# ltronchin/Gan-track

Hardware: AMD Instinct MI355X
Metric: imgs/sec at 256^2 bs32/GPU StyleGAN2-ADA training (+ sec/kimg) (higher is better)
Workload: dtype fp16+fp32 (fp16 at the 4 highest resolutions, fp32 below; f32 accumulate); 1 GPU; StyleGAN2-ADA train iteration, 256x256 1-ch, c_dim 2, cbase 16384, map 8, Gmain+Dmain / Greg every 4 / Dreg every 16, ADA geometric p=0.2; global_batch=32, batch_gpu=32, resolution=256, parallelism=dp1

## Files before the change

### gan-track_amd/csrc/conv3x3.hip

```cpp
#include "sg2_common.h"

#include <algorithm>
#include <atomic>
#include <type_traits>

namespace sg2 {
namespace {

constexpr int CK = 32;
constexpr int BN = 64;
constexpr int PX = CK;

__device__ __forceinline__ int swz64(int p, int q) { return p * 64 + ((q ^ ((p >> 1) & 2)) << 4); }

struct Conv3Args {
    const void* x;
    const void* w;
    void* y;
    void* y_raw;
    const float* in_scale;
    const float* out_scale;
    const void* noise;
    const float* bias;
    const void* dot_src;
    float* dot_out;
    float noise_gain, alpha, gain, clamp;
    int act;
    int N, H, W, Cin, Cout;
    int tiles_x, tiles_y;
    int OH, OW;
    const void* residual;
    int raw_act;
    float* det_dot;
    int edge_rx, edge_cy;
    int det_maxb;
};

__device__ __forceinline__ int p_chan(int P) { return (P >> 5) * 32 + 8 * ((P & 15) >> 2) + 4 * ((P >> 4) & 1) + (P & 3); }

template <typename T>
using v8 = typename std::conditional<std::is_same<T, bf16_t>::value, bf16x8, f16x8>::type;

template <typename T>
__device__ __forceinline__ f32x4 mma(v8<T> a, v8<T> b, f32x4 c) {
    if constexpr (std::is_same<T, bf16_t>::value)
        return __builtin_amdgcn_mfma_f32_16x16x32_bf16(a, b, c, 0, 0, 0);
    else
        return __builtin_amdgcn_mfma_f32_16x16x32_f16(a, b, c, 0, 0, 0);
}

template <typename T, int TW, bool SCALE_IN, bool EPI, int NBUF, int S = 1, bool DIR = false>
__global__ __launch_bounds__(256, 3 - NBUF) void conv3x3_halo_kernel(Conv3Args a) {
    static_assert(!DIR || S == 1, "the direct epilogue is the stride-1 form");
    constexpr int TH = S == 1 ? 256 / TW : 4;
    constexpr int PXW = TW * TH / 4, NFR = PXW / 16;
    constexpr int HW_ = S * (TW - 1) + 3, HH = S * (TH - 1) + 3, HP = HW_ * HH;
    constexpr int HEV = (HW_ + 1) / 2;
    constexpr int HALO = HP * PX;
    constexpr int WTS = 9 * BN * PX;
    constexpr int NH = (HP * 4 + 255) / 256;
    constexpr int NW = (9 * BN * 4) / 256;
    typedef T vec8 __attribute__((ext_vector_type(8)));

    extern __shared__ __attribute__((aligned(16))) char smem_raw[];
    T* smem = (T*)smem_raw;

    const int tid = threadIdx.x, lane = tid & 63, wave = tid >> 6;
    const int tile = blockIdx.x;
    const int n = tile / (a.tiles_x * a.tiles_y);
    const int tr = tile - n * a.tiles_x * a.tiles_y;
    const int ty0 = (tr / a.tiles_x) * TH, tx0 = (tr % a.tiles_x) * TW;
    const int o0 = blockIdx.y * BN;
    const T* __restrict__ x = (const T*)a.x;
    const T* __restrict__ w = (const T*)a.w;
    const int nchunks = (a.Cin + CK - 1) / CK;

    int h_src[NH], h_dst[NH];
    bool h_ok[NH];
#pragma unroll
    for (int i = 0; i < NH; ++i) {
        const int idx = tid + i * 256;
        const int p = idx >> 2, q = idx & 3;
        const int hy = p / HW_, hx = p - hy * HW_;
        const int iy = S == 1 ? ty0 - 1 + hy : 2 * ty0 + hy, ix = S == 1 ? tx0 - 1 + hx : 2 * tx0 + hx;
        h_ok[i] = p < HP && iy >= 0 && iy < a.H && ix >= 0 && ix < a.W;
        h_src[i] = h_ok[i] ? ((n * a.H + iy) * a.W + ix) : 0;
        const int pl = S == 1 ? p : hy * HW_ + ((hx & 1) ? HEV + (hx >> 1) : (hx >> 1));
        h_dst[i] = p < HP ? swz64(pl, q) : -1;
    }
    const int hq = (tid & 3) * 8;
    int w_src[NW], w_dst[NW];
    bool w_ok[NW];
#pragma unroll
    for (int i = 0; i < NW; ++i) {
        const int idx = tid + i * 256;
        const int r = idx >> 2;
        const int tap = r / BN, o = r - tap * BN;
        w_ok[i] = o0 + o < a.Cout;
        w_src[i] = (w_ok[i] ? (o0 + (DIR ? p_chan(o) : o)) : 0) * 9 + tap;
        w_dst[i] = swz64(tap * BN + o, idx & 3);
    }

    const __amdgpu_buffer_rsrc_t rxb = make_rsrc(x, (int64_t)a.N * a.H * a.W * a.Cin * (int64_t)sizeof(T));
    const __amdgpu_buffer_rsrc_t rwb = make_rsrc(w, (int64_t)a.Cout * 9 * a.Cin * (int64_t)sizeof(T));
    vec8 rh[NH], rw[NW];
    float4 sc0, sc1;
    auto gload = [&](int chunk) {
        const int c = chunk * CK + hq;
        const bool cok = c < a.Cin;
        const int cc = cok ? c : 0;
#pragma unroll
        for (int i = 0; i < NH; ++i)
            rh[i] = buf_load16<vec8>(rxb, h_ok[i] && cok ? (h_src[i] * a.Cin + c) * (int)sizeof(T) : -1);
#pragma unroll
        for (int i = 0; i < NW; ++i)
            rw[i] = buf_load16<vec8>(rwb, w_ok[i] && cok ? (w_src[i] * a.Cin + c) * (int)sizeof(T) : -1);
        if (SCALE_IN) {
            const float* sc = a.in_scale + (int64_t)n * a.Cin + cc;
            sc0 = *(const float4*)sc;
            sc1 = *(const float4*)(sc + 4);
        }
    };
    auto sstore = [&](int buf) {
        T* hb = smem + buf * (HALO + WTS);
        T* wb = hb + HALO;
        const float scl[8] = {sc0.x, sc0.y, sc0.z, sc0.w, sc1.x, sc1.y, sc1.z, sc1.w};
#pragma unroll
        for (int i = 0; i < NH; ++i) {
            if (h_dst[i] < 0) continue;
            vec8 v = rh[i];
            if (SCALE_IN) {
#pragma unroll
                for (int j = 0; j < 8; ++j) v[j] = (T)((float)v[j] * (float)(T)scl[j]);
            }
            *(vec8*)((char*)hb + h_dst[i]) = v;
        }
#pragma unroll
        for (int i = 0; i < NW; ++i) *(vec8*)((char*)wb + w_dst[i]) = rw[i];
    };

    const int lq = lane >> 4, l16 = lane & 15;
    int a_pos[NFR];
#pragma unroll
    for (int i = 0; i < NFR; ++i) {
        const int m = wave * PXW + i * 16 + l16;
        const int py = m / TW, px = m - py * TW;
        a_pos[i] = S * py * HW_ + px;
    }
    const int b_lane = swz64(l16, lq);

    f32x4 acc[NFR][4];
#pragma unroll
    for (int i = 0; i < NFR; ++i)
#pragma unroll
        for (int j = 0; j < 4; ++j) acc[i][j] = f32x4{0.f, 0.f, 0.f, 0.f};

    gload(0);
    sstore(0);
    __syncthreads();
    for (int ch = 0; ch < nchunks; ++ch) {
        const int cur = NBUF == 2 ? (ch & 1) : 0;
        const bool more = ch + 1 < nchunks;
        if (more) gload(ch + 1);
        const char* hb = (const char*)(smem + cur * (HALO + WTS));
        const char* wb = hb + HALO * sizeof(T) + b_lane;
#pragma unroll
        for (int ky = 0; ky < 3; ++ky) {
#pragma unroll
            for (int kx = 0; kx < 3; ++kx) {
                const int tap = ky * 3 + kx;
                const int toff = ky * HW_ + (S == 1 ? kx : ((kx & 1) ? HEV : (kx >> 1)));
                v8<T> af[NFR], bfr[4];
#pragma unroll
                for (int i = 0; i < NFR; ++i) af[i] = *(const v8<T>*)(hb + swz64(a_pos[i] + toff, lq));
#pragma unroll
                for (int j = 0; j < 4; ++j) bfr[j] = *(const v8<T>*)(wb + (tap * BN + j * 16) * 64);
#pragma unroll
                for (int i = 0; i < NFR; ++i)
#pragma unroll
                    for (int j = 0; j < 4; ++j) acc[i][j] = DIR ? mma<T>(bfr[j], af[i], acc[i][j]) : mma<T>(af[i], bfr[j], acc[i][j]);
            }
        }
        if (NBUF == 1 && more) __syncthreads();
        if (more) sstore(NBUF == 2 ? (cur ^ 1) : 0);
        __syncthreads();
    }

    if constexpr (DIR) {
        float dsc[2][8], bsc[2][8];
#pragma unroll
        for (int h = 0; h < 2; ++h)
#pragma unroll
            for (int e = 0; e < 8; ++e) {
                const int o = o0 + 32 * h + 8 * lq + e;
                dsc[h][e] = (EPI && a.out_scale) ? a.out_scale[(int64_t)n * a.Cout + o] : 1.f;
                bsc[h][e] = (EPI && a.bias) ? (float)(T)a.bias[o] : 0.f;
            }
        typedef T vec8d __attribute__((ext_vector_type(8)));
        const bool want_dot = a.dot_out != nullptr, atom = want_dot && !a.det_dot;
        float* red = (float*)smem;
        if (atom) {
            if (tid < BN) red[tid] = 0.f;
            __syncthreads();
        }
        float dacc[2][8];
#pragma unroll
        for (int h = 0; h < 2; ++h)
#pragma unroll
            for (int e = 0; e < 8; ++e) dacc[h][e] = 0.f;
        T* y = (T*)a.y;
        T* yr = (T*)a.y_raw;
        const T* dsrc = (const T*)a.dot_src;
        const T* nz = (const T*)a.noise;
#pragma unroll
        for (int i = 0; i < NFR; ++i) {
            const int m = wave * PXW + i * 16 + l16;
            const int py = m / TW, px = m - py * TW;
            const int oy = ty0 + py, ox = tx0 + px;
            const bool ok = oy < a.OH && ox < a.OW;
            const int64_t pix = ((int64_t)n * a.OH + (ok ? oy : 0)) * a.OW + (ok ? ox : 0);
            const float nv = (EPI && nz) ? (float)nz[pix] * a.noise_gain : 0.f;
#pragma unroll
            for (int h = 0; h < 2; ++h) {
                vec8d yv, rv;
#pragma unroll
                for (int e = 0; e < 8; ++e) {
                    float v = acc[i][2 * h + (e >> 2)][e & 3];
                    rv[e] = (T)v;
                    if (EPI) {
                        v = v * dsc[h][e] + nv + bsc[h][e];
                        if (a.act == 1) v = v > 0.f ? v : v * a.alpha;
                        v *= a.gain;
                        if (a.clamp >= 0.f) v = fminf(fmaxf(v, -a.clamp), a.clamp);
                    }
                    yv[e] = (T)v;
                }
                if (!ok) continue;
                const int64_t dst = pix * a.Cout + o0 + 32 * h + 8 * lq;
                *(vec8d*)(y + dst) = yv;
                if (yr) *(vec8d*)(yr + dst) = rv;
                if (want_dot) {
                    const vec8d sv = *(const vec8d*)(dsrc + dst);
#pragma unroll
                    for (int e = 0; e < 8; ++e) dacc[h][e] += (float)rv[e] * (float)sv[e];
                }
            }
        }
        if (want_dot) {
#pragma unroll
            for (int h = 0; h < 2; ++h)
#pragma unroll
                for (int e = 0; e < 8; ++e) {
                    float v = dacc[h][e];
                    v += __shfl_xor(v, 1);
                    v += __shfl_xor(v, 2);
                    v += __shfl_xor(v, 4);
                    v += __shfl_xor(v, 8);
                    if (l16 == 0) {
                        if (atom) atomicAdd(&red[32 * h + 8 * lq + e], v);
                        else red[wave * BN + 32 * h + 8 * lq + e] = v;
                    }
                }
            __syncthreads();
            if (tid < BN) {
                if (atom) atomicAdd(&a.dot_out[(int64_t)n * a.Cout + o0 + tid], red[tid]);
                else a.det_dot[(int64_t)tile * a.Cout + o0 + tid] = ((red[tid] + red[BN + tid]) + red[2 * BN + tid]) +
                                                                     red[3 * BN + tid];
            }
        }
        return;
    }
    float dsc[4], bsc[4];
#pragma unroll
    for (int j = 0; j < 4; ++j) {
        const int o = o0 + j * 16 + (lane & 15);
        const int oc = o < a.Cout ? o : 0;
        dsc[j] = (EPI && a.out_scale) ? a.out_scale[(int64_t)n * a.Cout + oc] : 1.f;
        bsc[j] = (EPI && a.bias) ? (float)(T)a.bias[oc] : 0.f;
    }
    constexpr int OS = BN + 8;
    constexpr int NPX = 4 * PXW;
    T* ot = smem;
    T* rt = smem + NPX * OS;
    float* red = (float*)(smem + 2 * NPX * OS);
    const T* nz = (const T*)a.noise;
    const bool want_raw = a.y_raw != nullptr;
    const bool want_dot = a.dot_out != nullptr;
    const bool keep_raw = want_raw || want_dot;
    if (want_dot && tid < BN) red[tid] = 0.f;
#pragma unroll
    for (int i = 0; i < NFR; ++i) {
#pragma unroll
        for (int r = 0; r < 4; ++r) {
            const int m = wave * PXW + i * 16 + 4 * (lane >> 4) + r;
            float nv = 0.f;
            if (EPI && nz) {
                const int py = m / TW, px = m - py * TW;
                const int oy = min(ty0 + py, a.OH - 1), ox = min(tx0 + px, a.OW - 1);
                nv = (float)nz[((int64_t)n * a.OH + oy) * a.OW + ox] * a.noise_gain;
            }
#pragma unroll
            for (int j = 0; j < 4; ++j) {
                float v = acc[i][j][r];
                if (keep_raw) rt[m * OS + j * 16 + (lane & 15)] = (T)v;
                if (EPI) {
                    v = v * dsc[j] + nv + bsc[j];
                    if (a.act == 1) v = v > 0.f ? v : v * a.alpha;
                    v *= a.gain;
                    if (a.clamp >= 0.f) v = fminf(fmaxf(v, -a.clamp), a.clamp);
                }
                ot[m * OS + j * 16 + (lane & 15)] = (T)v;
            }
        }
    }
    __syncthreads();
    typedef T vec8o __attribute__((ext_vector_type(8)));
    T* y = (T*)a.y;
    T* yr = (T*)a.y_raw;
    const T* dsrc = (const T*)a.dot_src;
    const bool cvec = (a.Cout % 8) == 0;
    float dacc[8];
#pragma unroll
    for (int e = 0; e < 8; ++e) dacc[e] = 0.f;
    const int c8 = (tid & 7) * 8;
#pragma unroll
    for (int k = 0; k < NPX / 32; ++k) {
        const int idx = tid + k * 256;
        const int m = idx >> 3;
        const int py = m / TW, px = m - py * TW;
        const int oy = ty0 + py, ox = tx0 + px;
        const int o = o0 + c8;
        if (oy >= a.OH || ox >= a.OW || o >= a.Cout) continue;
        const int64_t dst = (((int64_t)n * a.OH + oy) * a.OW + ox) * a.Cout + o;
        if (cvec) {
            vec8o yo = *(const vec8o*)(ot + m * OS + c8);
            if (a.residual) {
                if (want_raw && a.raw_act) *(vec8o*)(yr + dst) = yo;
                const vec8o rr = *(const vec8o*)((const T*)a.residual + dst);
#pragma unroll
                for (int e = 0; e < 8; ++e) yo[e] = (T)((float)yo[e] + (float)rr[e]);
            }
            *(vec8o*)(y + dst) = yo;
            if (want_raw && !a.raw_act) *(vec8o*)(yr + dst) = *(const vec8o*)(rt + m * OS + c8);
            if (want_dot) {
                const vec8o sv = *(const vec8o*)(dsrc + dst);
                const vec8o rv = *(const vec8o*)(rt + m * OS + c8);
#pragma unroll
                for (int e = 0; e < 8; ++e) dacc[e] += (float)rv[e] * (float)sv[e];
            }
        } else {
            for (int e = 0; e < 8 && o + e < a.Cout; ++e) {
                T yo = ot[m * OS + c8 + e];
                if (want_raw) yr[dst + e] = a.raw_act ? yo : rt[m * OS + c8 + e];
                if (a.residual) yo = (T)((float)yo + (float)((const T*)a.residual)[dst + e]);
                y[dst + e] = yo;
                if (want_dot) dacc[e] += (float)rt[m * OS + c8 + e] * (float)dsrc[dst + e];
            }
        }
    }
    if (want_dot && !a.det_dot) {
#pragma unroll
        for (int e = 0; e < 8; ++e) atomicAdd(&red[c8 + e], dacc[e]);
        __syncthreads();
        if (tid < BN && o0 + tid < a.Cout) atomicAdd(&a.dot_out[(int64_t)n * a.Cout + o0 + tid], red[tid]);
    } else if (want_dot) {
        float* part = (float*)smem;
        __syncthreads();
#pragma unroll
        for (int e = 0; e < 8; ++e) part[(tid >> 3) * BN + c8 + e] = dacc[e];
        __syncthreads();
        if (tid < BN && o0 + tid < a.Cout) {
            float v = 0.f;
            for (int r = 0; r < 32; ++r) v += part[r * BN + tid];
            a.det_dot[(int64_t)tile * a.Cout + o0 + tid] = v;
        }
    }
}

template <typename T, int TW, bool SI, bool EPI, int NBUF, int S = 1, bool DIR = false>
int launch3_k(const Conv3Args& a, hipStream_t s) {
    constexpr int TH = S == 1 ? 256 / TW : 4;
    size_t lds = NBUF * (size_t)((S * (TW - 1) + 3) * (S * (TH - 1) + 3) * PX + 9 * BN * PX) * sizeof(T);
    if (!DIR) lds = std::max(lds, (size_t)2 * TW * TH * (BN + 8) * sizeof(T) + BN * sizeof(float));
    auto kern = conv3x3_halo_kernel<T, TW, SI, EPI, NBUF, S, DIR>;
    static bool attr_set = false;
    if (!attr_set) {
        (void)hipFuncSetAttribute((const void*)kern, hipFuncAttributeMaxDynamicSharedMemorySize, (int)lds);
        attr_set = true;
    }
    dim3 grid(a.N * a.tiles_x * a.tiles_y, (a.Cout + BN - 1) / BN);
    if (a.dot_out && det_on()) {
        Conv3Args b = a;
        DetArena arena;
        const int tps = a.tiles_x * a.tiles_y;
        SG2_DET_GET(b.det_dot, arena, (int64_t)grid.x * a.Cout, "sg2_conv3x3");
        kern<<<grid, 256, lds, s>>>(b);
        if (int rc = launch_status("sg2_conv3x3")) return rc;
        hipError_t e = det_sum(a.dot_out, a.Cout, b.det_dot, (int64_t)tps * a.Cout, a.Cout, a.N, tps, a.Cout, arena, s,
                               det_assign());
        if (e) { set_error("sg2_conv3x3: det_sum"); return (int)e; }
        return 0;
    }
    kern<<<grid, 256, lds, s>>>(a);
    return launch_status("sg2_conv3x3");
}

template <typename T, int TW, bool SI, bool EPI, int NBUF, int S = 1>
int launch3(const Conv3Args& a, hipStream_t s) {
    if constexpr (S == 1) {
        const char* e = getenv("SG2_HALO_DIRECT");
        if ((!e || atoi(e) != 0) && a.Cout % BN == 0 && ((uintptr_t)a.y % 16) == 0 && ((uintptr_t)a.y_raw % 16) == 0 &&
            ((uintptr_t)a.dot_src % 16) == 0)
            return launch3_k<T, TW, SI, EPI, NBUF, 1, true>(a, s);
    }
    return launch3_k<T, TW, SI, EPI, NBUF, S, false>(a, s);
}

#ifndef SG2_DIAG
#define SG2_DIAG 0
#endif
constexpr int P_TW = 32, P_TH = 16, P_C = 64;
constexpr int P_HW = P_TW + 2, P_HH = P_TH + 2, P_HP = P_HW * P_HH;
constexpr int P_POS = CK * 2;
constexpr int P_WB = 2 * 9 * P_C * P_POS;
constexpr int P_HB = P_HP * P_POS;
constexpr int P_EB = (2 * P_C + P_TW * P_TH) * 4 + 16;
constexpr size_t P_LDS = (size_t)P_WB + 2 * P_HB + P_EB;
static_assert(P_WB % 256 == 0 && P_HB % 256 == 0, "swizzle assumes 256-byte aligned regions");

typedef unsigned int u32x4 __attribute__((ext_vector_type(4)));
__device__ __forceinline__ int swz(int pos, int q) { return pos * P_POS + ((q ^ ((pos >> 1) & 2)) << 4); }

template <typename T, bool SCALE_IN, bool EPI, bool DOT>
__global__ __launch_bounds__(512, 1) void conv3x3_c64p_kernel(Conv3Args a, int tiles_total) {
    constexpr int NT = 512;
    constexpr int NH = (P_HP * 4 + NT - 1) / NT;
    constexpr int NWL = 2 * 9 * P_C * 4 / NT;
    typedef T vec8 __attribute__((ext_vector_type(8)));
    typedef T vec4 __attribute__((ext_vector_type(4)));
    extern __shared__ __attribute__((aligned(16))) char smem_raw[];
    char* wlds = smem_raw;
    char* hlds = smem_raw + P_WB;
    float* blds = (float*)(smem_raw + P_WB + 2 * P_HB);
    float* dlds = blds + P_C;
    float* nlds = dlds + P_C;

    const int tid = threadIdx.x, lane = tid & 63, wave = tid >> 6;
    const int tiles_x = a.W / P_TW, tiles_y = a.H / P_TH;
    const int per_n = tiles_x * tiles_y;
    const int t_begin = (int)((int64_t)blockIdx.x * tiles_total / gridDim.x);
    const int t_end = (int)((int64_t)(blockIdx.x + 1) * tiles_total / gridDim.x);
    if (t_begin >= t_end) return;
    const __amdgpu_buffer_rsrc_t rxb = make_rsrc(a.x, (int64_t)a.N * a.H * a.W * P_C * (int64_t)sizeof(T));
    const __amdgpu_buffer_rsrc_t rwb = make_rsrc(a.w, (int64_t)P_C * 9 * P_C * (int64_t)sizeof(T));

#pragma unroll
    for (int k = 0; k < NWL; ++k) {
        const int idx = tid + k * NT;
        const int c = idx / (9 * P_C * 4), rem = idx - c * 9 * P_C * 4;
        const int r = rem >> 2, q = rem & 3, tap = r / P_C, row = r - tap * P_C;
        const int o = p_chan(row);
        const vec8 v = buf_load16<vec8>(rwb, ((o * 9 + tap) * P_C + c * CK + q * 8) * (int)sizeof(T));
        *(vec8*)(wlds + swz((c * 9 + tap) * P_C + row, q)) = v;
    }
    if (tid < P_C) blds[tid] = (EPI && a.bias) ? (float)(T)a.bias[tid] * a.gain : 0.f;

    int h_dy[NH], h_dx[NH], h_dst[NH];
#pragma unroll
    for (int i = 0; i < NH; ++i) {
        const int idx = tid + i * NT, p = idx >> 2, q = idx & 3;
        h_dy[i] = p / P_HW - 1;
        h_dx[i] = p % P_HW - 1;
        h_dst[i] = p < P_HP ? swz(p, q) : -1;
    }
    const int hq = (tid & 3) * 8;
    vec8 rh[NH];
    float4 s0, s1;
    const __amdgpu_buffer_rsrc_t rsc = make_rsrc(a.in_scale, SCALE_IN ? (int64_t)a.N * P_C * 4 : 0);
    auto tile_of = [&](int t, int& n, int& ty0, int& tx0) {
        n = t / per_n;
        const int tr = t - n * per_n;
        ty0 = (tr / tiles_x) * P_TH;
        tx0 = (tr % tiles_x) * P_TW;
    };
    auto gload = [&](int t, int c) {
        int n, ty0, tx0;
        tile_of(t, n, ty0, tx0);
// ... 1014 lines not shown
#pragma unroll
            for (int e = 0; e < 8; ++e) {
                const float cv = A[i][e >> 2][e & 3];
                if (RAW) rv[e] = (T)cv;
                float v = cv;
                if (EPI) {
                    v = fmaf(v, dd[e], nz[i] + bb[e]);
                    v = fmaxf(v, v * lr_alpha);
                    v = __builtin_amdgcn_fmed3f(v, -clampv, clampv);
                }
                yv[e] = (T)v;
            }
            const int dst = (pix * 32 + ch0) * (int)sizeof(T);
            __builtin_amdgcn_raw_buffer_store_b128(__builtin_bit_cast(u32x4, yv), ryb, dst, 0, 0);
            if (RAW) __builtin_amdgcn_raw_buffer_store_b128(__builtin_bit_cast(u32x4, rv), ryr, dst, 0, 0);
        }
    };
    auto mfma_tile = [&](f32x4 (&A)[NF][2], const char* hb) {
#pragma unroll
        for (int ky = 0; ky < 3; ++ky)
#pragma unroll
            for (int kx = 0; kx < 3; ++kx) {
                v8<T> pf[NF];
#pragma unroll
                for (int i = 0; i < NF; ++i)
                    pf[i] = *(const v8<T>*)(hb + boff[kx] + (((i >> 1) + ky) * Q_PITCH + (i & 1) * 16) * 64);
                const bool first = ky == 0 && kx == 0;
#pragma unroll
                for (int i = 0; i < NF; ++i)
#pragma unroll
                    for (int jj = 0; jj < 2; ++jj)
                        A[i][jj] = mma<T>(wf[jj][ky * 3 + kx], pf[i], first ? f32x4{0.f, 0.f, 0.f, 0.f} : A[i][jj]);
            }
    };

    issue(t_begin, 0, 0);
    wait_vm<0>();
    __builtin_amdgcn_s_waitcnt(0xc07f);
    __builtin_amdgcn_s_barrier();
    f32x4 acc[NF][2];
    int k = 0;
    for (int t = t_begin; t < t_end; ++t, ++k) {
        const int slot = k & 1;
        issue(min(t + 1, t_end - 1), slot ^ 1, (k + 1) % Q_NEPI);
        int n, ty, tx;
        tile_of(t, n, ty, tx);
        if (SI && n != cur_n) {
            cur_n = n;
            load_weights(n);
        }
        mfma_tile(acc, smem_raw + slot * Q_SLOT);
        float bb[8], dd[8], nz[NF];
        epi_table(k % Q_NEPI, bb, dd, nz);
        epi_store(acc, n, ty, tx, bb, dd, nz);
        wait_vm<S>();
        __builtin_amdgcn_s_waitcnt(0xc07f);
        __builtin_amdgcn_s_barrier();
    }
    wait_vm<0>();
}

template <typename T, bool SI, bool EPI, bool RAW>
int launch_c32r(const Conv3Args& a, hipStream_t s, int tiles, int grid, int band) {
    auto kern = conv3x3_c32r_kernel<T, SI, EPI, RAW>;
    static bool attr_set = false;
    if (!attr_set) {
        (void)hipFuncSetAttribute((const void*)kern, hipFuncAttributeMaxDynamicSharedMemorySize, (int)Q_LDS);
        attr_set = true;
    }
    kern<<<grid, 256, Q_LDS, s>>>(a, tiles, band);
    return launch_status("sg2_conv3x3 (c32 ring)");
}

template <typename T, bool SI, bool EPI>
int launch_c32r_raw(const Conv3Args& a, hipStream_t s) {
    const int tiles = a.N * (a.H / Q_TH) * (a.W / Q_TW);
    const int ty = a.H / Q_TH;
    const int band = ty % 4 == 0 ? 4 : (ty % 2 == 0 ? 2 : 1);
    const int grid = 2 * num_cus();
    return a.y_raw ? launch_c32r<T, SI, EPI, true>(a, s, tiles, grid, band)
                   : launch_c32r<T, SI, EPI, false>(a, s, tiles, grid, band);
}

constexpr int G_BM = 256, G_BN = 128, G_NS = 3;
constexpr int G_SLOT = (G_BM + G_BN) * 64;
constexpr int G_DMA = (G_BM + G_BN) / 16 / 4;
constexpr int G_ADMA = G_BM / 16 / 4;
constexpr size_t G_LDS = (size_t)G_NS * G_SLOT;

template <typename T, bool EPI>
__global__ __launch_bounds__(256, 2) void conv3x3_s2g_kernel(Conv3Args a, int m_tiles, int n_tiles) {
    typedef T vec8 __attribute__((ext_vector_type(8)));
    extern __shared__ __attribute__((aligned(16))) char smem_raw[];
    const int tid = threadIdx.x, lane = tid & 63;
    const int wave = __builtin_amdgcn_readfirstlane(tid >> 6);
    const int l16 = lane & 15, q = lane >> 4;
    const int t = (int)(blockIdx.x % 8) * (int)(gridDim.x / 8) + (int)(blockIdx.x / 8);
    if (t >= m_tiles * n_tiles) return;
    const int mt = t / n_tiles, nt = t - mt * n_tiles;
    const int OHW = a.OH * a.OW, M = a.N * OHW;
    const int m0 = mt * G_BM, n0 = nt * G_BN;
    const int nk = 9 * (a.Cin / 32);
    const __amdgpu_buffer_rsrc_t rxb = make_rsrc(a.x, (int64_t)a.N * a.H * a.W * a.Cin * 2);
    const __amdgpu_buffer_rsrc_t rwb = make_rsrc(a.w, (int64_t)a.Cout * 9 * a.Cin * 2);

    int dbase[G_DMA];
#pragma unroll
    for (int u = 0; u < G_DMA; ++u) {
        const int r = (u * 4 + wave) * 16 + (lane >> 2);
        const int j = (lane & 3) ^ ((r >> 1) & 2);
        if (u < G_ADMA) {
            const int m = m0 + r;
            if (m < M) {
                const int n = m / OHW, rem = m - n * OHW, oy = rem / a.OW, ox = rem - oy * a.OW;
                dbase[u] = (((n * a.H + 2 * oy) * a.W + 2 * ox) * a.Cin + j * 8) * 2;
            } else {
                dbase[u] = -1;
            }
        } else {
            dbase[u] = ((n0 + p_chan(r - G_BM)) * 9 * a.Cin + j * 8) * 2;
        }
    }
    auto issue = [&](int step, int slot) {
        const int tap = step % 9, c = step / 9;
        const int ky = tap / 3, kx = tap - ky * 3;
        const int aoff = ((ky * a.W + kx) * a.Cin + c * 32) * 2, boff = (tap * a.Cin + c * 32) * 2;
        char* sb = smem_raw + slot * G_SLOT;
#pragma unroll
        for (int u = 0; u < G_DMA; ++u) {
            if (u < G_ADMA) {
                const int off = dbase[u] < 0 ? -1 : dbase[u] + aoff;
                __builtin_amdgcn_raw_ptr_buffer_load_lds(rxb, (lds_ptr_t)(sb + (u * 4 + wave) * 1024), 16, off, 0, 0, 0);
            } else {
                __builtin_amdgcn_raw_ptr_buffer_load_lds(rwb, (lds_ptr_t)(sb + (u * 4 + wave) * 1024), 16, dbase[u] + boff,
                                                         0, 0, 0);
            }
        }
    };

    const int wm = wave >> 1, wn = wave & 1;
    const int sw = ((q ^ ((l16 >> 1) & 2)) << 4) + l16 * 64;
    f32x4 acc[4][8];
#pragma unroll
    for (int i = 0; i < 4; ++i)
#pragma unroll
        for (int j = 0; j < 8; ++j) acc[i][j] = f32x4{0.f, 0.f, 0.f, 0.f};

#pragma unroll
    for (int st = 0; st < G_NS - 1; ++st)
        if (st < nk) issue(st, st);
    for (int step = 0; step < nk; ++step) {
        if (step + G_NS - 2 < nk) wait_vm<(G_NS - 2) * G_DMA>();
        else wait_vm<0>();
        __builtin_amdgcn_s_waitcnt(0xc07f);
        __builtin_amdgcn_s_barrier();
        if (step + G_NS - 1 < nk) issue(step + G_NS - 1, (step + G_NS - 1) % G_NS);
        const char* sb = smem_raw + (step % G_NS) * G_SLOT + sw;
        v8<T> wf[4], pf[8];
#pragma unroll
        for (int jc = 0; jc < 4; ++jc) wf[jc] = *(const v8<T>*)(sb + (G_BM + wn * 64 + jc * 16) * 64);
#pragma unroll
        for (int jp = 0; jp < 8; ++jp) pf[jp] = *(const v8<T>*)(sb + (wm * 128 + jp * 16) * 64);
#pragma unroll
        for (int jp = 0; jp < 8; ++jp)
#pragma unroll
            for (int jc = 0; jc < 4; ++jc) acc[jc][jp] = mma<T>(wf[jc], pf[jp], acc[jc][jp]);
// ... 53 lines not shown
    const int grid = (m_tiles * n_tiles + 7) / 8 * 8;
    auto kern = conv3x3_s2g_kernel<T, EPI>;
    static bool attr_set = false;
    if (!attr_set) {
        (void)hipFuncSetAttribute((const void*)kern, hipFuncAttributeMaxDynamicSharedMemorySize, (int)G_LDS);
        attr_set = true;
    }
    kern<<<grid, 256, G_LDS, s>>>(a, m_tiles, n_tiles);
    return launch_status("sg2_conv3x3_s2 (s2g)");
}

template <typename T>
int dispatch(Conv3Args& a, hipStream_t s, int stride) {
    const bool si = a.in_scale != nullptr;
    const bool epi = a.out_scale || a.noise || a.bias || a.act != 0 || a.gain != 1.f || a.clamp >= 0.f;
    if (a.dot_out) {
        hipError_t e = zero_acc(a.dot_out, (size_t)a.N * a.Cout * sizeof(float), s);
        if (e != hipSuccess) { set_error("sg2_conv3x3: memset failed"); return (int)e; }
    }
    if (stride == 2) {
        const char* eg = getenv("SG2_S2G");
        if ((!eg || atoi(eg) != 0) && !si && !a.noise && !a.dot_out && a.Cin % 32 == 0 && a.Cout % G_BN == 0 &&
            a.OW >= 32 && (int64_t)a.N * a.OH * a.OW * a.Cout * 2 < 0x7fff0000ll &&
            ((uintptr_t)a.y % 16) == 0 && ((uintptr_t)a.y_raw % 16) == 0 && ((uintptr_t)a.residual % 16) == 0 &&
            (!epi || a.gain > 0.f)) {
            if (epi) return launch_s2g<T, true>(a, s);
            return launch_s2g<T, false>(a, s);
        }
        a.tiles_x = (a.OW + 31) / 32;
        a.tiles_y = (a.OH + 3) / 4;
        if (si) { if (epi) return launch3<T, 32, true, true, 1, 2>(a, s); return launch3<T, 32, true, false, 1, 2>(a, s); }
        if (epi) return launch3<T, 32, false, true, 1, 2>(a, s);
        return launch3<T, 32, false, false, 1, 2>(a, s);
    }
    static const bool persist = [] { const char* e = getenv("SG2_HALO_PERSIST"); return !e || atoi(e) != 0; }();
    {
        const char* e32 = getenv("SG2_C32_RING");
        const bool ring32 = !e32 || atoi(e32) != 0;
        const int tiles = a.H % Q_TH == 0 && a.W % Q_TW == 0 ? a.N * (a.H / Q_TH) * (a.W / Q_TW) : 0;
        const int grid = 2 * num_cus();
        if (ring32 && !a.dot_out && a.Cin == 32 && a.Cout == 32 && tiles >= 2 * grid && tiles <= 128 * grid &&
            a.N < 4096 && a.H / Q_TH < 1024 && a.W / Q_TW < 1024 &&
            (int64_t)a.N * a.H * a.W * 32 * (int64_t)sizeof(T) < 0x7fff0000ll &&
            ((uintptr_t)a.y % 16) == 0 && ((uintptr_t)a.y_raw % 16) == 0 && ((uintptr_t)a.noise % 16) == 0 &&
            ((uintptr_t)a.out_scale % 16) == 0 && ((uintptr_t)a.in_scale % 16) == 0 && (a.W * (int)sizeof(T)) % 16 == 0 &&
            (!epi || (a.gain > 0.f && (a.act == 0 || (a.alpha >= 0.f && a.alpha <= 1.f))))) {
            if (si) { if (epi) return launch_c32r_raw<T, true, true>(a, s); return launch_c32r_raw<T, true, false>(a, s); }
            if (epi) return launch_c32r_raw<T, false, true>(a, s);
            return launch_c32r_raw<T, false, false>(a, s);
        }
    }
    const char* ring_env = getenv("SG2_C64_RING");
    const int ring = ring_env ? atoi(ring_env) : 49;
    const int rth = (ring == 4 || ring == 44 || ring == 46 || ring == 49) ? 4 : 8;
    if (ring && !a.dot_out && a.Cin == P_C && a.Cout == P_C && a.H % rth == 0 && a.W % R_TW == 0 &&
        ((uintptr_t)a.y % 16) == 0 && ((uintptr_t)a.y_raw % 16) == 0 && ((uintptr_t)a.noise % 16) == 0 &&
        ((uintptr_t)a.out_scale % 16) == 0 && ((uintptr_t)a.in_scale % 16) == 0 &&
        (!epi || (a.gain > 0.f && (a.act == 0 || (a.alpha >= 0.f && a.alpha <= 1.f))))) {
        const int tiles = a.N * (a.H / rth) * (a.W / R_TW);
        const int grid = (rth == 4 ? 2 : 1) * num_cus();
        if (tiles >= 2 * grid && tiles <= 128 * grid && a.N < 4096 && a.H / rth < 1024 && a.W / R_TW < 1024 &&
            (int64_t)a.N * a.H * a.W * 64 * (int64_t)sizeof(T) < 0x7fff0000ll) {
            const int form = (ring == 84 || ring == 44 || ring == 46 || ring == 49) ? ring : rth;
            if (si) { if (epi) return launch_c64r_form<T, true, true>(a, s, form); return launch_c64r_form<T, true, false>(a, s, form); }
            if (epi) return launch_c64r_form<T, false, true>(a, s, form);
            return launch_c64r_form<T, false, false>(a, s, form);
        }
    }
    if (persist && a.Cin == P_C && a.Cout == P_C && a.H % P_TH == 0 && a.W % P_TW == 0 &&
        (!epi || (a.gain > 0.f && (a.act == 0 || (a.alpha >= 0.f && a.alpha <= 1.f))))) {
        const int tiles = a.N * (a.H / P_TH) * (a.W / P_TW);
        if (tiles >= 2 * num_cus()) {
            const int grid = num_cus();
            if (si) { if (epi) return launch_c64p_dot<T, true, true>(a, s, tiles, grid); return launch_c64p_dot<T, true, false>(a, s, tiles, grid); }
            if (epi) return launch_c64p_dot<T, false, true>(a, s, tiles, grid);
            return launch_c64p_dot<T, false, false>(a, s, tiles, grid);
        }
    }
    const int TW = a.W >= 32 ? 32 : 16;
    a.tiles_x = (a.W + TW - 1) / TW;
    a.tiles_y = (a.H + (256 / TW) - 1) / (256 / TW);
    static const int force_nbuf = [] { const char* e = getenv("SG2_HALO_NBUF"); return e ? atoi(e) : 0; }();
    const int nbuf = force_nbuf ? force_nbuf : 1;
#define L3(TWV, SIV, EPIV) return nbuf == 1 ? launch3<T, TWV, SIV, EPIV, 1>(a, s) : launch3<T, TWV, SIV, EPIV, 2>(a, s)
    if (TW == 32) {
        if (si) { if (epi) L3(32, true, true); else L3(32, true, false); }
        else { if (epi) L3(32, false, true); else L3(32, false, false); }
    } else {
        if (si) { if (epi) L3(16, true, true); else L3(16, true, false); }
        else { if (epi) L3(16, false, true); else L3(16, false, false); }
    }
#undef L3
}

constexpr int U_TW = 16, U_TH = 8, U_CELLS = U_TW * U_TH;
constexpr int U_HW = U_TW + 1, U_HH = U_TH + 1, U_HP = U_HW * U_HH;
constexpr int U_HB = ((U_HP * 64 + 255) / 256) * 256;
constexpr int U_WB = 9 * BN * 64;
constexpr int U_OS = BN + 8;
constexpr size_t U_LDS = (size_t)U_HB + U_WB;
static_assert((size_t)U_CELLS * U_OS * 2 <= U_LDS, "epilogue tile fits the staging buffer");

template <int EDGE> struct UpGeom {
    static constexpr int TW = EDGE == 0 ? U_TW : (EDGE == 1 ? 128 : 1);
    static constexpr int HR = EDGE == 1 ? 1 : (EDGE == 0 ? U_TH : 128) + 1;
    static constexpr int HC = EDGE == 2 ? 1 : TW + 1;
    static constexpr int HP = HR * HC;
    static constexpr int NT = EDGE == 0 ? 9 : 3;
    __device__ static constexpr int tap(int t) { return EDGE == 0 ? t : (EDGE == 1 ? 6 + t : 2 + 3 * t); }
};
static_assert(((UpGeom<1>::HP * 64 + 255) / 256) * 256 + 3 * BN * 64 <= U_LDS &&
              ((UpGeom<2>::HP * 64 + 255) / 256) * 256 + 3 * BN * 64 <= U_LDS, "edge strips fit the staging buffer");

template <typename T, bool SCALE_IN, int EDGE>
__device__ __forceinline__ void up2_tile(const Conv3Args& a, int n, int i0, int j0, char* smem_raw) {
    using G = UpGeom<EDGE>;
    constexpr int NH = (G::HP * 4 + 255) / 256;
    constexpr int NW = (G::NT * BN * 4) / 256;
    constexpr int HB = ((G::HP * 64 + 255) / 256) * 256;
    typedef T vec8 __attribute__((ext_vector_type(8)));
    char* hl = smem_raw;
    char* wl = smem_raw + HB;

    const int tid = threadIdx.x, lane = tid & 63, wave = tid >> 6;
    const int o0 = blockIdx.y * BN;
    const int OH = 2 * a.H + 1, OW = 2 * a.W + 1;
    const int nchunks = a.Cin / CK;
    const __amdgpu_buffer_rsrc_t rxb = make_rsrc(a.x, (int64_t)a.N * a.H * a.W * a.Cin * (int64_t)sizeof(T));
    const __amdgpu_buffer_rsrc_t rwb = make_rsrc(a.w, (int64_t)a.Cout * 9 * a.Cin * (int64_t)sizeof(T));
    const int hq = (tid & 3) * 8;

    vec8 rh[NH], rw[NW];
    float4 sc0, sc1;
    auto gload = [&](int chunk) {
        const int c = chunk * CK + hq;
#pragma unroll
        for (int k = 0; k < NH; ++k) {
            const int p = (tid + k * 256) >> 2;
            const int iy = i0 - 1 + p / G::HC, ix = j0 - 1 + p % G::HC;
            const bool ok = (p < G::HP) & ((unsigned)iy < (unsigned)a.H) & ((unsigned)ix < (unsigned)a.W);
            rh[k] = buf_load16<vec8>(rxb, ok ? (((n * a.H + iy) * a.W + ix) * a.Cin + c) * (int)sizeof(T) : -1);
        }
#pragma unroll
        for (int k = 0; k < NW; ++k) {
            const int r = (tid + k * 256) >> 2, t = r / BN, o = r - t * BN;
            rw[k] = buf_load16<vec8>(rwb, o0 + o < a.Cout ? (((o0 + o) * 9 + G::tap(t)) * a.Cin + c) * (int)sizeof(T)
                                                          : -1);
        }
        if (SCALE_IN) {
            const float* sc = a.in_scale + (int64_t)n * a.Cin + c;
            sc0 = *(const float4*)sc;
            sc1 = *(const float4*)(sc + 4);
        }
    };
    auto sstore = [&]() {
        const float scl[8] = {sc0.x, sc0.y, sc0.z, sc0.w, sc1.x, sc1.y, sc1.z, sc1.w};
#pragma unroll
        for (int k = 0; k < NH; ++k) {
            const int p = (tid + k * 256) >> 2;
            if (k * 256 + 256 > G::HP * 4 && p >= G::HP) continue;
            vec8 v = rh[k];
            if (SCALE_IN) {
#pragma unroll
                for (int e = 0; e < 8; ++e) v[e] = (T)((float)v[e] * (float)(T)scl[e]);
            }
            *(vec8*)(hl + swz64(p, tid & 3)) = v;
// ... 198 lines not shown
```

Before: 777.3 imgs/s.

## Add double-buffered direct-to-LDS DMA halo conv3x3 kernel for 32-wide tiles

Adds a new 3x3 conv kernel that loads the input halo and weights into LDS with buffer_load_lds DMA. Loads are double-buffered and split into parts across the ky loop, so the next chunk's transfer overlaps the MFMA work on the current one. Input scaling is applied in place in LDS, and the output goes through the direct register epilogue, which is factored into a shared helper. The kernel is on by default for 32-wide tiles with suitable channel counts, replacing the older register-staged halo path. In exchange it adds more barriers per chunk and layout and alignment conditions that must hold.

```diff
diff --git a/gan-track_amd/csrc/conv3x3.hip b/gan-track_amd/csrc/conv3x3.hip
--- a/gan-track_amd/csrc/conv3x3.hip
+++ b/gan-track_amd/csrc/conv3x3.hip
@@ -49,6 +49,94 @@
         return __builtin_amdgcn_mfma_f32_16x16x32_f16(a, b, c, 0, 0, 0);
 }
 
+template <typename T, int TW, int NFR, bool EPI>
+__device__ __forceinline__ void halo_direct_epilogue(const Conv3Args& a, const f32x4 (&acc)[NFR][4], float* red, int n,
+                                                     int tile, int ty0, int tx0, int o0) {
+    constexpr int PXW = NFR * 16;
+    const int tid = threadIdx.x, lane = tid & 63, wave = tid >> 6;
+    const int lq = lane >> 4, l16 = lane & 15;
+    float dsc[2][8], bsc[2][8];
+#pragma unroll
+    for (int h = 0; h < 2; ++h)
+#pragma unroll
+        for (int e = 0; e < 8; ++e) {
+            const int o = o0 + 32 * h + 8 * lq + e;
+            dsc[h][e] = (EPI && a.out_scale) ? a.out_scale[(int64_t)n * a.Cout + o] : 1.f;
+            bsc[h][e] = (EPI && a.bias) ? (float)(T)a.bias[o] : 0.f;
+        }
+    typedef T vec8d __attribute__((ext_vector_type(8)));
+    const bool want_dot = a.dot_out != nullptr, atom = want_dot && !a.det_dot;
+    if (atom) {
+        if (tid < BN) red[tid] = 0.f;
+        __syncthreads();
+    }
+    float dacc[2][8];
+#pragma unroll
+    for (int h = 0; h < 2; ++h)
+#pragma unroll
+        for (int e = 0; e < 8; ++e) dacc[h][e] = 0.f;
+    T* y = (T*)a.y;
+    T* yr = (T*)a.y_raw;
+    const T* dsrc = (const T*)a.dot_src;
+    const T* nz = (const T*)a.noise;
+#pragma unroll
+    for (int i = 0; i < NFR; ++i) {
+        const int m = wave * PXW + i * 16 + l16;
+        const int py = m / TW, px = m - py * TW;
+        const int oy = ty0 + py, ox = tx0 + px;
+        const bool ok = oy < a.OH && ox < a.OW;
+        const int64_t pix = ((int64_t)n * a.OH + (ok ? oy : 0)) * a.OW + (ok ? ox : 0);
+        const float nv = (EPI && nz) ? (float)nz[pix] * a.noise_gain : 0.f;
+#pragma unroll
+        for (int h = 0; h < 2; ++h) {
+            vec8d yv, rv;
+#pragma unroll
+            for (int e = 0; e < 8; ++e) {
+                float v = acc[i][2 * h + (e >> 2)][e & 3];
+                rv[e] = (T)v;
+                if (EPI) {
+                    v = v * dsc[h][e] + nv + bsc[h][e];
+                    if (a.act == 1) v = v > 0.f ? v : v * a.alpha;
+                    v *= a.gain;
+                    if (a.clamp >= 0.f) v = fminf(fmaxf(v, -a.clamp), a.clamp);
+                }
+                yv[e] = (T)v;
+            }
+            if (!ok) continue;
+            const int64_t dst = pix * a.Cout + o0 + 32 * h + 8 * lq;
+            *(vec8d*)(y + dst) = yv;
+            if (yr) *(vec8d*)(yr + dst) = rv;
+            if (want_dot) {
+                const vec8d sv = *(const vec8d*)(dsrc + dst);
+#pragma unroll
+                for (int e = 0; e < 8; ++e) dacc[h][e] += (float)rv[e] * (float)sv[e];
+            }
+        }
+    }
+    if (want_dot) {
+#pragma unroll
+        for (int h = 0; h < 2; ++h)
+#pragma unroll
+            for (int e = 0; e < 8; ++e) {
+                float v = dacc[h][e];
+                v += __shfl_xor(v, 1);
+                v += __shfl_xor(v, 2);
+                v += __shfl_xor(v, 4);
+                v += __shfl_xor(v, 8);
+                if (l16 == 0) {
+                    if (atom) atomicAdd(&red[32 * h + 8 * lq + e], v);
+                    else red[wave * BN + 32 * h + 8 * lq + e] = v;
+                }
+            }
+        __syncthreads();
+        if (tid < BN) {
+            if (atom) atomicAdd(&a.dot_out[(int64_t)n * a.Cout + o0 + tid], red[tid]);
+            else a.det_dot[(int64_t)tile * a.Cout + o0 + tid] = ((red[tid] + red[BN + tid]) + red[2 * BN + tid]) +
+                                                                 red[3 * BN + tid];
+        }
+    }
+}
+
 template <typename T, int TW, bool SCALE_IN, bool EPI, int NBUF, int S = 1, bool DIR = false>
 __global__ __launch_bounds__(256, 3 - NBUF) void conv3x3_halo_kernel(Conv3Args a) {
     static_assert(!DIR || S == 1, "the direct epilogue is the stride-1 form");
@@ -187,87 +275,7 @@
     }
 
     if constexpr (DIR) {
-        float dsc[2][8], bsc[2][8];
-#pragma unroll
-        for (int h = 0; h < 2; ++h)
-#pragma unroll
-            for (int e = 0; e < 8; ++e) {
-                const int o = o0 + 32 * h + 8 * lq + e;
-                dsc[h][e] = (EPI && a.out_scale) ? a.out_scale[(int64_t)n * a.Cout + o] : 1.f;
-                bsc[h][e] = (EPI && a.bias) ? (float)(T)a.bias[o] : 0.f;
-            }
-        typedef T vec8d __attribute__((ext_vector_type(8)));
-        const bool want_dot = a.dot_out != nullptr, atom = want_dot && !a.det_dot;
-        float* red = (float*)smem;
-        if (atom) {
-            if (tid < BN) red[tid] = 0.f;
-            __syncthreads();
-        }
-        float dacc[2][8];
-#pragma unroll
-        for (int h = 0; h < 2; ++h)
-#pragma unroll
-            for (int e = 0; e < 8; ++e) dacc[h][e] = 0.f;
-        T* y = (T*)a.y;
-        T* yr = (T*)a.y_raw;
-        const T* dsrc = (const T*)a.dot_src;
-        const T* nz = (const T*)a.noise;
-#pragma unroll
-        for (int i = 0; i < NFR; ++i) {
-            const int m = wave * PXW + i * 16 + l16;
-            const int py = m / TW, px = m - py * TW;
-            const int oy = ty0 + py, ox = tx0 + px;
-            const bool ok = oy < a.OH && ox < a.OW;
-            const int64_t pix = ((int64_t)n * a.OH + (ok ? oy : 0)) * a.OW + (ok ? ox : 0);
-            const float nv = (EPI && nz) ? (float)nz[pix] * a.noise_gain : 0.f;
-#pragma unroll
-            for (int h = 0; h < 2; ++h) {
-                vec8d yv, rv;
-#pragma unroll
-                for (int e = 0; e < 8; ++e) {
-                    float v = acc[i][2 * h + (e >> 2)][e & 3];
-                    rv[e] = (T)v;
-                    if (EPI) {
-                        v = v * dsc[h][e] + nv + bsc[h][e];
-                        if (a.act == 1) v = v > 0.f ? v : v * a.alpha;
-                        v *= a.gain;
-                        if (a.clamp >= 0.f) v = fminf(fmaxf(v, -a.clamp), a.clamp);
-                    }
-                    yv[e] = (T)v;
-                }
-                if (!ok) continue;
-                const int64_t dst = pix * a.Cout + o0 + 32 * h + 8 * lq;
-                *(vec8d*)(y + dst) = yv;
-                if (yr) *(vec8d*)(yr + dst) = rv;
-                if (want_dot) {
-                    const vec8d sv = *(const vec8d*)(dsrc + dst);
-#pragma unroll
-                    for (int e = 0; e < 8; ++e) dacc[h][e] += (float)rv[e] * (float)sv[e];
-                }
-            }
-        }
-        if (want_dot) {
-#pragma unroll
-            for (int h = 0; h < 2; ++h)
-#pragma unroll
-                for (int e = 0; e < 8; ++e) {
-                    float v = dacc[h][e];
-                    v += __shfl_xor(v, 1);
-                    v += __shfl_xor(v, 2);
-                    v += __shfl_xor(v, 4);
-                    v += __shfl_xor(v, 8);
-                    if (l16 == 0) {
-                        if (atom) atomicAdd(&red[32 * h + 8 * lq + e], v);
-                        else red[wave * BN + 32 * h + 8 * lq + e] = v;
-                    }
-                }
-            __syncthreads();
-            if (tid < BN) {
-                if (atom) atomicAdd(&a.dot_out[(int64_t)n * a.Cout + o0 + tid], red[tid]);
-                else a.det_dot[(int64_t)tile * a.Cout + o0 + tid] = ((red[tid] + red[BN + tid]) + red[2 * BN + tid]) +
-                                                                     red[3 * BN + tid];
-            }
-        }
+        halo_direct_epilogue<T, TW, NFR, EPI>(a, acc, (float*)smem, n, tile, ty0, tx0, o0);
         return;
     }
     float dsc[4], bsc[4];
@@ -377,17 +385,8 @@
     }
 }
 
-template <typename T, int TW, bool SI, bool EPI, int NBUF, int S = 1, bool DIR = false>
-int launch3_k(const Conv3Args& a, hipStream_t s) {
-    constexpr int TH = S == 1 ? 256 / TW : 4;
-    size_t lds = NBUF * (size_t)((S * (TW - 1) + 3) * (S * (TH - 1) + 3) * PX + 9 * BN * PX) * sizeof(T);
-    if (!DIR) lds = std::max(lds, (size_t)2 * TW * TH * (BN + 8) * sizeof(T) + BN * sizeof(float));
-    auto kern = conv3x3_halo_kernel<T, TW, SI, EPI, NBUF, S, DIR>;
-    static bool attr_set = false;
-    if (!attr_set) {
-        (void)hipFuncSetAttribute((const void*)kern, hipFuncAttributeMaxDynamicSharedMemorySize, (int)lds);
-        attr_set = true;
-    }
+template <typename K>
+int launch_halo_tiles(K kern, size_t lds, const Conv3Args& a, hipStream_t s) {
     dim3 grid(a.N * a.tiles_x * a.tiles_y, (a.Cout + BN - 1) / BN);
     if (a.dot_out && det_on()) {
         Conv3Args b = a;
@@ -403,6 +402,20 @@
     }
     kern<<<grid, 256, lds, s>>>(a);
     return launch_status("sg2_conv3x3");
+}
+
+template <typename T, int TW, bool SI, bool EPI, int NBUF, int S = 1, bool DIR = false>
+int launch3_k(const Conv3Args& a, hipStream_t s) {
+    constexpr int TH = S == 1 ? 256 / TW : 4;
+    size_t lds = NBUF * (size_t)((S * (TW - 1) + 3) * (S * (TH - 1) + 3) * PX + 9 * BN * PX) * sizeof(T);
+    if (!DIR) lds = std::max(lds, (size_t)2 * TW * TH * (BN + 8) * sizeof(T) + BN * sizeof(float));
+    auto kern = conv3x3_halo_kernel<T, TW, SI, EPI, NBUF, S, DIR>;
+    static bool attr_set = false;
+    if (!attr_set) {
+        (void)hipFuncSetAttribute((const void*)kern, hipFuncAttributeMaxDynamicSharedMemorySize, (int)lds);
+        attr_set = true;
+    }
+    return launch_halo_tiles(kern, lds, a, s);
 }
 
 template <typename T, int TW, bool SI, bool EPI, int NBUF, int S = 1>
@@ -1583,6 +1596,155 @@
                    : launch_c32r<T, SI, EPI, false>(a, s, tiles, grid, band);
 }
 
+constexpr int D_TW = 32, D_TH = 8, D_PITCH = 36;
+constexpr int D_HPOS = (D_TH + 2) * D_PITCH;
+constexpr int D_HDMA = 6;
+constexpr int D_HSLOT = D_HDMA * 4 * 1024;
+constexpr int D_WDMA = 3;
+constexpr int D_WSLOT = 3 * BN * 64;
+constexpr int D_SCIN = 1024;
+constexpr size_t D_LDS = 2 * D_HSLOT + 2 * D_WSLOT + D_SCIN * 2 + 4 * BN * sizeof(float);
+static_assert(D_HPOS * 64 <= D_HSLOT && D_WSLOT == D_WDMA * 4 * 1024 && 2 * D_LDS <= 160 * 1024, "halo DMA LDS");
+
+template <typename T, bool SCALE_IN, bool EPI>
+__global__ __launch_bounds__(256, 2) void conv3x3_halo_dma_kernel(Conv3Args a) {
+    constexpr int NFR = 4;
+    constexpr int HPARTS = SCALE_IN ? 2 : 3, HPD = D_HDMA / HPARTS;
+    extern __shared__ __attribute__((aligned(16))) char smem_raw[];
+    char* hs = smem_raw;
+    char* ws = smem_raw + 2 * D_HSLOT;
+    T* stab = (T*)(ws + 2 * D_WSLOT);
+    float* red = (float*)(ws + 2 * D_WSLOT + D_SCIN * 2);
+
+    const int tid = threadIdx.x, lane = tid & 63;
+    const int wave = __builtin_amdgcn_readfirstlane(tid >> 6);
+    const int lq = lane >> 4, l16 = lane & 15;
+    const int tile = blockIdx.x;
+    const int n = tile / (a.tiles_x * a.tiles_y);
+    const int tr = tile - n * a.tiles_x * a.tiles_y;
+    const int ty0 = (tr / a.tiles_x) * D_TH, tx0 = (tr % a.tiles_x) * D_TW;
+    const int o0 = blockIdx.y * BN;
+    const int nchunks = a.Cin / CK;
+
+    const __amdgpu_buffer_rsrc_t rxb = make_rsrc(a.x, (int64_t)a.N * a.H * a.W * a.Cin * (int64_t)sizeof(T));
+    const __amdgpu_buffer_rsrc_t rwb = make_rsrc(a.w, (int64_t)a.Cout * 9 * a.Cin * (int64_t)sizeof(T));
+    int hbase[D_HDMA], wbase[D_WDMA];
+#pragma unroll
+    for (int u = 0; u < D_HDMA; ++u) {
+        const int p = (u * 4 + wave) * 16 + (lane >> 2);
+        const int j = (lane & 3) ^ ((p >> 1) & 2);
+        const int hy = p / D_PITCH, hx = p - hy * D_PITCH;
+        const int iy = ty0 - 1 + hy, ix = tx0 - 1 + hx;
+        const bool ok = p < D_HPOS && hx < D_TW + 2 && (unsigned)iy < (unsigned)a.H && (unsigned)ix < (unsigned)a.W;
+        hbase[u] = ok ? (((n * a.H + iy) * a.W + ix) * a.Cin + j * 8) * (int)sizeof(T) : (int)0x80000000;
+    }
+#pragma unroll
+    for (int u = 0; u < D_WDMA; ++u) {
+        const int r = (u * 4 + wave) * 16 + (lane >> 2);
+        const int j = (lane & 3) ^ ((r >> 1) & 2);
+        wbase[u] = (((o0 + p_chan(r & (BN - 1))) * 9 + u) * a.Cin + j * 8) * (int)sizeof(T);
+    }
+    auto issue_w = [&](int chunk, int ky, int slot) {
+        const int off = (ky * 3 * a.Cin + chunk * CK) * (int)sizeof(T);
+#pragma unroll
+        for (int u = 0; u < D_WDMA; ++u)
+            __builtin_amdgcn_raw_ptr_buffer_load_lds(rwb, (lds_ptr_t)(ws + slot * D_WSLOT + (u * 4 + wave) * 1024), 16,
+                                                     wbase[u] + off, 0, 0, 0);
+    };
+    auto issue_h = [&](int chunk, int part, int slot) {
+        const int off = chunk * CK * (int)sizeof(T);
+#pragma unroll
+        for (int v = 0; v < HPD; ++v) {
+            const int u = part * HPD + v;
+            __builtin_amdgcn_raw_ptr_buffer_load_lds(rxb, (lds_ptr_t)(hs + slot * D_HSLOT + (u * 4 + wave) * 1024), 16,
+                                                     hbase[u] + off, 0, 0, 0);
+        }
+    };
+    auto scale_h = [&](int chunk, int part, int slot) {
+        typedef T vec8 __attribute__((ext_vector_type(8)));
+        const int j = (lane & 3) ^ (((lane >> 4) & 1) << 1);
+        const vec8 sv = *(const vec8*)(stab + chunk * CK + j * 8);
+#pragma unroll
+        for (int v = 0; v < HPD; ++v) {
+            vec8* p = (vec8*)(hs + slot * D_HSLOT + ((part * HPD + v) * 4 + wave) * 1024 + lane * 16);
+            vec8 x8 = *p;
+#pragma unroll
+            for (int e = 0; e < 8; ++e) x8[e] = (T)((float)x8[e] * (float)sv[e]);
+            *p = x8;
+        }
+    };
+
+    int aoff[3][2];
+#pragma unroll
+    for (int kx = 0; kx < 3; ++kx)
+#pragma unroll
+        for (int par = 0; par < 2; ++par) {
+            const int v = l16 + kx;
+            aoff[kx][par] = (wave * 2 * D_PITCH + v) * 64 + ((lq ^ ((((v >> 2) & 1) ^ par) << 1)) << 4);
+        }
+    const int b_lane = swz64(l16, lq);
+
+    f32x4 acc[NFR][4];
+#pragma unroll
+    for (int i = 0; i < NFR; ++i)
+#pragma unroll
+        for (int j = 0; j < 4; ++j) acc[i][j] = f32x4{0.f, 0.f, 0.f, 0.f};
+
+#pragma unroll
+    for (int part = 0; part < HPARTS; ++part) issue_h(0, part, 0);
+    issue_w(0, 0, 0);
+    if (SCALE_IN) {
+        for (int c = tid; c < a.Cin; c += 256) stab[c] = (T)a.in_scale[(int64_t)n * a.Cin + c];
+        __syncthreads();
+        wait_vm<0>();
+#pragma unroll
+        for (int part = 0; part < HPARTS; ++part) scale_h(0, part, 0);
+    }
+    for (int ch = 0; ch < nchunks; ++ch) {
+        const bool more = ch + 1 < nchunks;
+        const char* hb = hs + (ch & 1) * D_HSLOT;
+#pragma unroll
+        for (int ky = 0; ky < 3; ++ky) {
+            const int wslot = (ch + ky) & 1;
+            wait_vm<0>();
+            __builtin_amdgcn_s_waitcnt(0xc07f);
+            __builtin_amdgcn_s_barrier();
+            if (ky < 2) issue_w(ch, ky + 1, wslot ^ 1);
+            else if (more) issue_w(ch + 1, 0, wslot ^ 1);
+            if (more && ky < HPARTS) issue_h(ch + 1, ky, (ch + 1) & 1);
+            const char* wb = ws + wslot * D_WSLOT + b_lane;
+#pragma unroll
+            for (int kx = 0; kx < 3; ++kx) {
+                v8<T> af[NFR], bfr[4];
+#pragma unroll
+                for (int i = 0; i < NFR; ++i) {
+                    const int row = (i >> 1) + ky;
+                    af[i] = *(const v8<T>*)(hb + aoff[kx][row & 1] + (row * D_PITCH + (i & 1) * 16) * 64);
+                }
+#pragma unroll
+                for (int j = 0; j < 4; ++j) bfr[j] = *(const v8<T>*)(wb + (kx * BN + j * 16) * 64);
+#pragma unroll
+                for (int i = 0; i < NFR; ++i)
+#pragma unroll
+                    for (int j = 0; j < 4; ++j) acc[i][j] = mma<T>(bfr[j], af[i], acc[i][j]);
+            }
+            if (SCALE_IN && more && ky >= 1) scale_h(ch + 1, ky - 1, (ch + 1) & 1);
+        }
+    }
+    halo_direct_epilogue<T, D_TW, NFR, EPI>(a, acc, red, n, tile, ty0, tx0, o0);
+}
+
+template <typename T, bool SI, bool EPI>
+int launch_halo_dma(const Conv3Args& a, hipStream_t s) {
+    auto kern = conv3x3_halo_dma_kernel<T, SI, EPI>;
+    static bool attr_set = false;
+    if (!attr_set) {
+        (void)hipFuncSetAttribute((const void*)kern, hipFuncAttributeMaxDynamicSharedMemorySize, (int)D_LDS);
+        attr_set = true;
+    }
+    return launch_halo_tiles(kern, D_LDS, a, s);
+}
+
 constexpr int G_BM = 256, G_BN = 128, G_NS = 3;
 constexpr int G_SLOT = (G_BM + G_BN) * 64;
 constexpr int G_DMA = (G_BM + G_BN) / 16 / 4;
@@ -1802,6 +1964,19 @@
     a.tiles_y = (a.H + (256 / TW) - 1) / (256 / TW);
     static const int force_nbuf = [] { const char* e = getenv("SG2_HALO_NBUF"); return e ? atoi(e) : 0; }();
     const int nbuf = force_nbuf ? force_nbuf : 1;
+    {
+        const char* ed = getenv("SG2_HALO_DMA");
+        const char* e1 = getenv("SG2_HALO_DIRECT");
+        if ((!ed || atoi(ed) != 0) && (!e1 || atoi(e1) != 0) && !force_nbuf && TW == 32 && a.Cin % CK == 0 &&
+            a.Cout % BN == 0 && a.Cin <= 16384 && (!si || a.Cin <= D_SCIN) &&
+            ((uintptr_t)a.y % 16) == 0 && ((uintptr_t)a.y_raw % 16) == 0 && ((uintptr_t)a.dot_src % 16) == 0 &&
+            (int64_t)a.N * a.H * a.W * a.Cin * (int64_t)sizeof(T) < 0x7fff0000ll &&
+            (int64_t)a.N * a.H * a.W * a.Cout * (int64_t)sizeof(T) < 0x7fff0000ll) {
+            if (si) { if (epi) return launch_halo_dma<T, true, true>(a, s); return launch_halo_dma<T, true, false>(a, s); }
+            if (epi) return launch_halo_dma<T, false, true>(a, s);
+            return launch_halo_dma<T, false, false>(a, s);
+        }
+    }
 #define L3(TWV, SIV, EPIV) return nbuf == 1 ? launch3<T, TWV, SIV, EPIV, 1>(a, s) : launch3<T, TWV, SIV, EPIV, 2>(a, s)
     if (TW == 32) {
         if (si) { if (epi) L3(32, true, true); else L3(32, true, false); }
```

Result: faster. 786.5 imgs/s, median of 6 (+1.2%).
